# fgvieira/ngsDist

Hardware: AMD Instinct MI355X
Metric: pair-distances/sec (higher is better)
Workload: dtype f64

## Files before the change

include/ngsdist_amd.h:

```cpp
#ifndef NGSDIST_AMD_H
#define NGSDIST_AMD_H

#include <stdint.h>

#ifdef __cplusplus
extern "C" {
#endif

#define NGD_ABI_VERSION 6

#define NGD_OK 0
#define NGD_E_INVALID (-1)
#define NGD_E_NODEVICE (-2)
#define NGD_E_HIP (-3)
#define NGD_E_NOMEM (-4)
#define NGD_E_MODEL (-5)
#define NGD_E_NAN (-6)

#define NGD_KERNEL_AUTO 0
#define NGD_KERNEL_STREAM 1
#define NGD_KERNEL_MFMA 2
#define NGD_KERNEL_EM_FAITHFUL 3
#define NGD_KERNEL_EM_FAST 4
#define NGD_KERNEL_EM_TABLE 5
// ... 98 lines not shown
#define NGD_OPT_STAGE_RING 11
#define NGD_OPT_EAGER_FULL 12
#define NGD_OPT_WIN_PLAN 13
#define NGD_OPT_WIN_MAX_BYTES 14
#define NGD_OPT_EM_EXACT 15
#define NGD_OPT_EM_EXACT_CAP 16
#define NGD_OPT_UNIT_SKIP 17
#define NGD_OPT_EM_EXACT_WIN 18
#define NGD_OPT_NJ_MAX_BYTES 19
#define NGD_OPT_MDS_MAX_BYTES 20
#define NGD_OPT_DEBUG_FORGE_JOB 100
int ngd_set_option(ngd_engine *e, int option, uint64_t value);

int ngd_last_timing(const ngd_engine *e, ngd_timing *t);
int ngd_last_plain_pass(const ngd_engine *e, uint64_t *kgroups);
int ngd_image_mode(const ngd_engine *e, int *fixup);
typedef struct ngd_fixup_info {
  uint64_t flagged, recomputed, skipped;
  double ms;
  uint64_t by_pass;
} ngd_fixup_info;
int ngd_last_fixup(const ngd_engine *e, ngd_fixup_info *info);
typedef struct ngd_spill_timing {
  double ms_weights;
  double ms_terms;
  double ms_sanitize;
  double ms_contract;
  uint64_t chunks;
  uint64_t sites;
  uint64_t unit_sites;
// ... 183 lines not shown
```

ngsdist_amd/_lib.py:

```python
import ctypes as C
import os
import sys

_HERE = os.path.dirname(os.path.abspath(__file__))
LIB_PATH = os.environ.get("NGSDIST_AMD_LIB") or os.path.join(_HERE, "libngsdist_amd.so")


class NgdConfig(C.Structure):
    _fields_ = [
        ("n_ind", C.c_uint64),
        ("n_sites", C.c_uint64),
        ("score", C.c_double * 9),
        ("pairwise_del", C.c_int32),
        ("indep_geno", C.c_int32),
        ("device", C.c_int32),
        ("kernel", C.c_int32),
        ("shard_rank", C.c_uint32),
        ("shard_world", C.c_uint32),
        ("variant", C.c_uint32),
        ("n_slices", C.c_uint32),
        ("wg_target", C.c_uint32),
        ("exact_shapes", C.c_uint32),
        ("single_image", C.c_uint32),
        ("second_image_mib", C.c_uint32),
# ... 34 lines not shown

class NgdEmExactInfo(C.Structure):
    _fields_ = [("noted", C.c_uint64), ("changed", C.c_uint64), ("passes", C.c_uint64), ("ms", C.c_double)]


class NgdEmExactEntry(C.Structure):
    _fields_ = [("i1", C.c_uint32), ("i2", C.c_uint32), ("site", C.c_uint64), ("t_dev", C.c_uint32), ("t_ref", C.c_uint32),
                ("c_dev", C.c_double), ("c_ref", C.c_double)]


EXPORTS = [
    "ngd_last_error", "ngd_abi_version", "ngd_device_count", "ngd_create", "ngd_destroy",
    "ngd_upload_sites", "ngd_upload_ind_major", "ngd_commit", "ngd_stage_acquire", "ngd_stage_submit",
    "ngd_upload_raw_sites", "ngd_synth_fill", "ngd_synth_fill_range", "ngd_run", "ngd_run_mult", "ngd_run_mult_device",
    "ngd_run_device", "ngd_run_batch", "ngd_run_batch_device", "ngd_run_mult_batch",
    "ngd_run_mult_batch_device", "ngd_run_job", "ngd_run_job_device", "ngd_run_job_dist", "ngd_run_batch_dist", "ngd_run_mult_batch_dist", "ngd_fetch_matrix", "ngd_drop_caches", "ngd_set_option", "ngd_last_timing", "ngd_last_plain_pass", "ngd_last_spill_timing", "ngd_last_fixup", "ngd_image_mode", "ngd_last_shader_clock", "ngd_last_em_work", "ngd_finish", "ngd_finish_stream", "ngd_format_matrix", "ngd_taus_seed", "ngd_taus_get",
    "ngd_taus_uniform", "ngd_boot_block_map", "ngd_n_pairs", "ngd_pair_index", "ngd_device_bytes", "ngd_device_memory", "ngd_shard_of_pair", "ngd_shard_map",
    "ngd_score_congruence", "ngd_run_windows", "ngd_run_windows_device", "ngd_run_windows_dist", "ngd_last_windows",
    "ngd_window_ranges", "ngd_run_windows_job", "ngd_run_windows_job_device", "ngd_run_windows_job_dist",
    "ngd_window_ranges_bp", "ngd_window_boot_maps", "ngd_run_windows_job_var", "ngd_run_windows_job_var_device",
    "ngd_run_windows_job_var_dist",
    "ngd_last_em_exact", "ngd_em_exact_entries", "ngd_em2_site",
    "ngd_n_group_pairs", "ngd_group_pair_index", "ngd_group_cells", "ngd_set_groups", "ngd_group_means_device",
    "ngd_run_job_groups", "ngd_run_windows_groups", "ngd_run_windows_job_var_groups", "ngd_last_groups_ms",
    "ngd_boot_stats_max_rep", "ngd_boot_stats_host", "ngd_boot_stats_device", "ngd_boot_stats_values_device",
    "ngd_run_job_stats", "ngd_run_windows_job_var_stats", "ngd_run_job_groups_stats", "ngd_run_windows_job_var_groups_stats",
    "ngd_last_boot_stats_ms",
    "ngd_nj_max_ind", "ngd_nj_host", "ngd_nj_values_device", "ngd_nj_device", "ngd_run_job_nj", "ngd_run_windows_nj",
    "ngd_run_windows_job_var_nj", "ngd_last_nj_ms", "ngd_nj_support", "ngd_nj_newick",
    "ngd_mds_max_ind", "ngd_mds_max_dim", "ngd_mds_host", "ngd_mds_coords", "ngd_mds_values_device", "ngd_mds_device",
    "ngd_run_job_mds", "ngd_run_windows_mds", "ngd_run_windows_job_var_mds", "ngd_last_mds_ms",
# ... 46 lines not shown
    L.ngd_run_batch.argtypes = [vp, u64p, C.c_uint32, u64, u64, dp, u64p]
    L.ngd_run_batch_device.argtypes = [vp, u64p, C.c_uint32, u64, u64, vp, vp]
    L.ngd_run_mult_batch.argtypes = [vp, u32p, C.c_uint32, u64, u64, dp, u64p]
    L.ngd_run_job.argtypes = [vp, u64p, C.c_uint32, u64, u64, dp, u64p]
    L.ngd_run_job_device.argtypes = [vp, u64p, C.c_uint32, u64, u64, vp, vp]
    L.ngd_fetch_matrix.argtypes = [vp, C.c_uint32, dp, u64p]
    L.ngd_run_job_dist.argtypes = [vp, u64p, C.c_uint32, u64, u64, u64, u64, dp]
    L.ngd_run_batch_dist.argtypes = [vp, u64p, C.c_uint32, u64, u64, u64, u64, dp]
    L.ngd_run_mult_batch_dist.argtypes = [vp, u32p, C.c_uint32, u64, u64, u64, u64, dp]
    L.ngd_run_mult_batch_device.argtypes = [vp, u32p, C.c_uint32, u64, u64, vp, vp]
    L.ngd_drop_caches.argtypes = [vp]
    L.ngd_set_option.argtypes = [vp, C.c_int, u64]
    L.ngd_last_timing.argtypes = [vp, C.POINTER(NgdTiming)]
    if hasattr(L, "ngd_last_plain_pass"):
        L.ngd_last_plain_pass.argtypes = [vp, u64p]
    L.ngd_last_spill_timing.argtypes = [vp, C.POINTER(NgdSpillTiming)]
    L.ngd_last_fixup.argtypes = [vp, C.POINTER(NgdFixupInfo)]
    L.ngd_image_mode.argtypes = [vp, C.POINTER(C.c_int)]
    L.ngd_image_mode.restype = C.c_int
    L.ngd_last_em_work.argtypes = [vp, u64p, u64p]
    L.ngd_last_shader_clock.argtypes = [vp, dp]
    L.ngd_finish.argtypes = [dp, u64p, u64, u64, u64, dp]
    L.ngd_finish_stream.argtypes = [dp, u64p, u64, u64, u64, dp, u64p]
    L.ngd_format_matrix.argtypes = [dp, u64, C.POINTER(C.c_char_p), C.c_char_p, u64, C.c_uint32]
    L.ngd_format_matrix.restype = C.c_int64
    L.ngd_device_memory.argtypes = [C.c_int, u64p, u64p]
    L.ngd_taus_seed.argtypes = [u32p, u64]
    L.ngd_taus_seed.restype = None
    L.ngd_taus_get.argtypes = [u32p]
    L.ngd_taus_get.restype = C.c_uint32
# ... 93 lines not shown
```

ngsdist_amd/csrc/engine.hip:

```cpp
#include "ngd_engine.h"

extern "C" {

const char *ngd_last_error(void) { return g_err.c_str(); }
int ngd_abi_version(void) { return NGD_ABI_VERSION; }

uint64_t ngd_n_pairs(uint64_t n_ind) { return n_ind * (n_ind - 1) / 2; }
uint64_t ngd_pair_index(uint64_t n_ind, uint64_t i1, uint64_t i2) { return ngd_pair_idx(n_ind, i1, i2); }
uint64_t ngd_device_bytes(const ngd_engine *e) { return e ? e->dev_bytes : 0; }

int ngd_run_device(ngd_engine *e, const uint64_t *block_map, uint64_t n_blocks, uint64_t block_size,
                   void *d_sum, void *d_cnt) {
  if (!d_sum || !d_cnt) return fail(NGD_E_INVALID, "ngd_run_device: null output");
  return run_impl(e, block_map, nullptr, block_map ? 1 : 0, false, n_blocks, block_size, (double *)d_sum,
                  (unsigned long long *)d_cnt);
}

int ngd_run_mult_device(ngd_engine *e, const uint32_t *mult, uint64_t n_blocks, uint64_t block_size, void *d_sum,
                        void *d_cnt) {
  if (!d_sum || !d_cnt || !mult) return fail(NGD_E_INVALID, "ngd_run_mult_device: null argument");
  return run_impl(e, nullptr, mult, 1, false, n_blocks, block_size, (double *)d_sum, (unsigned long long *)d_cnt);
}

int ngd_run_mult(ngd_engine *e, const uint32_t *mult, uint64_t n_blocks, uint64_t block_size, double *sum,
// ... 115 lines not shown
      if (e->pin_sites || e->committed) return fail(NGD_E_INVALID, "ngd_set_option: NGD_OPT_EAGER_FULL before the first ngd_stage_acquire");
      if (value && e->opt_em_exact) return fail(NGD_E_INVALID, "ngd_set_option: NGD_OPT_EAGER_FULL and NGD_OPT_EM_EXACT refuse each other (the eager pass does not note)");
      e->opt_eager = value != 0 && eager_supported(e);
      break;
    case NGD_OPT_STAGE_PIECE_MIB:
    case NGD_OPT_STAGE_RING:
      if (e->pin_sites) return fail(NGD_E_INVALID, "ngd_set_option: the staging ring exists already (set before the first ngd_stage_acquire)");
      if (option == NGD_OPT_STAGE_RING) {
        if (value < 2 || value > ngd_engine::RING) return fail(NGD_E_INVALID, "ngd_set_option: NGD_OPT_STAGE_RING is 2 .. 8");
        e->opt_stage_ring = value;
      } else {
        if (value < 1 || value > 1024) return fail(NGD_E_INVALID, "ngd_set_option: NGD_OPT_STAGE_PIECE_MIB is 1 .. 1024");
        e->opt_stage_piece_mib = value;
      }
      break;
    case NGD_OPT_UNIT_SKIP: e->opt_unit_skip = value != 0; break;
    case NGD_OPT_DEBUG_FORGE_JOB: {
      const char *hook = getenv("NGD_ENABLE_TEST_HOOKS");
      if (!hook || strcmp(hook, "1") != 0)
        return fail(NGD_E_INVALID, "ngd_set_option: NGD_OPT_DEBUG_FORGE_JOB is a test hook (set NGD_ENABLE_TEST_HOOKS=1)");
      if (e->kernel != NGD_KERNEL_MFMA || !e->d_jobs) return fail(NGD_E_INVALID, "ngd_set_option: no MFMA job list");
      HIPCHK(hipSetDevice(e->device));
      ngd_job j;
      HIPCHK(hipMemcpy(&j, e->d_jobs, sizeof(j), hipMemcpyDeviceToHost));
      j.rows = (uint8_t)(value & 7); j.cols = (uint8_t)((value >> 3) & 7); j.tri = (uint8_t)((value >> 6) & 1);
      HIPCHK(hipMemcpy(e->d_jobs, &j, sizeof(j), hipMemcpyHostToDevice));
      break;
    }
    default: return fail(NGD_E_INVALID, "ngd_set_option: unknown option");
  }
  return NGD_OK;
// ... 32 lines not shown
  return e->congruent ? 2 : e->single_image ? 1 : 3;
}

int ngd_last_spill_timing(const ngd_engine *e, ngd_spill_timing *t) {
  if (!e || !t) return fail(NGD_E_INVALID, "ngd_last_spill_timing: null argument");
  *t = e->spill_timing;
  return NGD_OK;
}

int ngd_last_plain_pass(const ngd_engine *e, uint64_t *kgroups) {
  if (!e || !kgroups) return fail(NGD_E_INVALID, "ngd_last_plain_pass: null argument");
  *kgroups = e->plain_kg;
  return NGD_OK;
}

int ngd_last_timing(const ngd_engine *e, ngd_timing *t) {
  if (!e || !t) return fail(NGD_E_INVALID, "ngd_last_timing: null argument");
  *t = e->timing;
  return NGD_OK;
}

}
```

ngsdist_amd/csrc/engine_plans.hip:

```cpp
#include "ngd_engine.h"

struct pass_slices {
  const uint32_t *w = nullptr, *kgl = nullptr;
  uint64_t sites_eff = 0;
  uint32_t n_ks = 0;
  uint64_t per_slice = 0, kg_lim = 0;
  double *slab = nullptr;
  uint64_t k_per_slice = 0;
  uint32_t w_stride = 0;
  bool note = false;
  const uint64_t *seg = nullptr;
};

static ngd_mfma_launch slices_launch(const ngd_engine *e, const pass_slices &p, const double *d_w_plain) {
  ngd_mfma_launch l;
  l.PA = e->PA;
  l.d_wk = p.k_per_slice ? e->blk.wslice : (p.w ? e->d_wk : d_w_plain);
  l.n_ks = p.n_ks; l.kg_per_slice = p.per_slice; l.n_kg_eff = p.kg_lim;
  l.k_per_slice = p.k_per_slice; l.w_slice_stride = p.w_stride;
  if (p.seg) { l.d_wk = e->blk.wslice; l.d_seg = p.seg; l.w_slice_stride = 1; l.k_per_slice = 0; }
  l.slab = p.slab;
  return l;
}

// ... 232 lines not shown
  int rc = pass_once(e, mult, mult_max, n_blocks, block_size, n_drawn, d_sum, d_cnt, add_timing, note);
  if (rc || !note) return rc;
  bool again = false;
  if ((rc = em_exact_finish(e, d_sum, &again))) return rc;
  if (again) {
    if ((rc = pass_once(e, mult, mult_max, n_blocks, block_size, n_drawn, d_sum, d_cnt, add_timing, true))) return rc;
    if ((rc = em_exact_finish(e, d_sum, &again))) return rc;
    if (again) return fail(NGD_E_HIP, "NGD_OPT_EM_EXACT: internal -- the second pass noted more than the first counted");
    e->exact_info.passes = 2;
  }
  return NGD_OK;
}

static int partials_impl(ngd_engine *e, const uint32_t *mult , const unsigned long long *drawn,
                         uint32_t n_rep, uint64_t n_blocks, uint64_t block_size, double *d_sum,
                         unsigned long long *d_cnt, bool *feasible, bool note = false) {
  const ngd_geom &g = e->g;
  const uint64_t n_pairs = ngd_n_pairs(g.n_ind);
  const uint64_t n_eff = n_blocks * block_size;
  const uint64_t plane = (uint64_t)g.n_pad * g.n_pad;
  const bool mfma = e->kernel == NGD_KERNEL_MFMA;
  const bool pdel = e->cfg.pairwise_del != 0;
  *feasible = false;
  if (e->kernel == NGD_KERNEL_STREAM || !e->opt_boot_partials) return NGD_OK;
  const bool unaligned = mfma && block_size % 4 != 0;
  if (unaligned && !e->opt_boot_unaligned) return NGD_OK;
  if (n_blocks >= (1ull << 31)) return NGD_OK;
  const uint64_t unit = mfma ? 3 * block_size / 4 : block_size;
  const bool cached = !note && e->blk.has_sums(block_size, n_blocks);
  uint64_t sub = 1, nks = 0;
  if (cached) {
    sub = e->blk.sub;
    nks = e->blk.nks;
  } else {
    const uint32_t tiles_n = mfma ? std::max(1u, e->n_wg / (e->exact_shapes && e->exact_shapes < 3 ? 4 : 1))
                                  : e->kernel == NGD_KERNEL_EM_TABLE ? e->n_tiles64 : e->n_tiles16;
    const uint64_t want = e->opt_boot_wg;
    while (!unaligned && tiles_n && (uint64_t)tiles_n * n_blocks * sub < want && unit % (sub * 2) == 0 &&
           unit / (sub * 2) >= 32)
      sub *= 2;
    nks = n_blocks * sub;
    if (mfma) nks = (nks + 7) / 8 * 8;
  }
  if (nks >= (1ull << 31)) return NGD_OK;
  const uint64_t elems = nks * plane, c_elems = pdel ? n_blocks * plane : 0;
  const bool c_cached = !pdel || e->blk.has_counts(block_size, n_blocks);
  if (!cached || !c_cached) {
    size_t free_b = 0, total_b = 0;
    HIPCHK(hipMemGetInfo(&free_b, &total_b));
    const uint64_t need = elems * 8 + c_elems * 4;
    const uint64_t have = e->blk.bytes();
    const uint64_t budget = e->opt_boot_max_bytes ? e->opt_boot_max_bytes : (uint64_t)((free_b + have) / 100 * 85);
    if (need > budget) return NGD_OK;
// ... 20 lines not shown
  }
  *feasible = true;
  if (e->out.on && out_trace()) fprintf(stderr, "[out] plan settled %.3f ms into the call\n", out_now() - e->out.t_call);

  HIPCHK(hipEventRecord(e->ev[0], e->st));
  uint32_t launches = 0;
  HIPCHK(hipEventRecord(e->ev[1], e->st));
  if (!cached) {
    int rc = e->blk.borrow_sums().ensure(e, elems);
    if (rc) return rc;
    e->blk.nks = (uint32_t)nks;
    e->blk.sub = (uint32_t)sub;
    e->blk.per_slice = unit / sub;
    pass_slices ps;
    ps.sites_eff = n_eff; ps.n_ks = e->blk.nks; ps.slab = e->blk.sums();
    if (unaligned && e->congruent) {
      std::vector<uint64_t> tab;
      tab.reserve((size_t)e->blk.nks * NGD_SEG_STRIDE);
      uint64_t wkg = 0, max_wkg = 0;
      for (uint64_t b = 0; b < n_blocks; b++) {
        const uint64_t s_lo = b * block_size, s_hi = s_lo + block_size;
        const uint64_t kg0 = ngd_kg_lo(s_lo, 1), kg1 = ngd_kg_hi(s_hi, 1), n_wkg = kg1 - kg0 + 1 + NGD_KG_TAIL;
        tab.insert(tab.end(), {kg0, kg1, wkg, s_lo, s_hi});
        wkg += n_wkg;
        max_wkg = std::max(max_wkg, n_wkg);
      }
      for (uint64_t k = n_blocks; k < e->blk.nks; k++) tab.insert(tab.end(), {0, 0, wkg, 0, 0});
      max_wkg = std::max<uint64_t>(max_wkg, 1 + NGD_KG_TAIL);
      rc = e->blk.wslice.ensure(e, (wkg + 1 + NGD_KG_TAIL) * 4);
      if (!rc) rc = e->d_segtab.ensure(e, tab.size());
      if (rc) return rc;
      HIPCHK(hipMemcpy(e->d_segtab, tab.data(), tab.size() * 8, hipMemcpyHostToDevice));
      ngd_launch_seg_weights(e->st, e->d_segtab, e->blk.nks, max_wkg, e->sc.d, e->blk.wslice);
      ps.kg_lim = g.n_kg; ps.seg = e->d_segtab;
    } else if (unaligned) {
      const uint32_t w_stride = (uint32_t)((3 * block_size + 3) / 4 + 1 + NGD_KG_TAIL);
      rc = e->blk.wslice.ensure(e, (uint64_t)e->blk.nks * w_stride * 4);
      if (rc) return rc;
      ngd_launch_slice_weights(e->st, e->blk.nks, w_stride, 3 * block_size, 3 * n_eff, e->blk.wslice);
      ps.kg_lim = (3 * n_eff + 3) / 4; ps.k_per_slice = 3 * block_size; ps.w_stride = w_stride;
    } else {
      if (note && (rc = em_exact_begin(e))) return rc;
      ps.per_slice = e->blk.per_slice; ps.kg_lim = mfma ? 3 * n_eff / 4 : 0; ps.note = note;
    }
    rc = launch_accumulate(e, ps);
    if (rc) return rc;
    HIPCHK(hipGetLastError());
    if (!note) e->blk.sums_filled(block_size, n_blocks);
    launches = 1;
  }
  HIPCHK(hipEventRecord(e->ev[2], e->st));

  const uint32_t stride = (n_rep + ngd_reduce_chunk(n_rep) - 1) / ngd_reduce_chunk(n_rep) * ngd_reduce_chunk(n_rep);
  const uint64_t n_slices = n_blocks * sub;
  std::vector<double> W(n_slices * stride, 0.0);
  for (uint32_t r = 0; r < n_rep; r++)
    for (uint64_t b = 0; b < n_blocks; b++) {
      const double m = (double)mult[(uint64_t)r * n_blocks + b];
      if (m != 0.0)
        for (uint64_t q = 0; q < sub; q++) W[(b * sub + q) * stride + r] = m;
    }
  int rc = e->d_W.ensure(e, W.size());
  if (rc) return rc;
  HIPCHK(hipMemcpyAsync(e->d_W, W.data(), W.size() * 8, hipMemcpyHostToDevice, e->st));
  if ((rc = zero_outputs(e, n_rep, d_sum, d_cnt, false))) return rc;
  const bool fix = e->SM != nullptr && mfma;
  const ngd_fix_flags ff{e->d_fixlist, e->d_fixcount, e->d_fixseen, e->fix_cap};
  std::vector<double> thr;
  if (fix) {
    thr.resize(n_rep);
    for (uint32_t r = 0; r < n_rep; r++) thr[r] = NGD_FIX_MEAN * (double)drawn[r];
    rc = e->d_fixthr.ensure(e, (uint64_t)n_rep);
    if (rc) return rc;
    HIPCHK(hipMemcpyAsync(e->d_fixthr, thr.data(), (uint64_t)n_rep * 8, hipMemcpyHostToDevice, e->st));
    HIPCHK(hipMemsetAsync(e->d_fixcount, 0, sizeof(uint32_t), e->st));
    HIPCHK(hipMemsetAsync(e->d_fixseen, 0, (n_pairs / 32 + 1) * sizeof(uint32_t), e->st));
  }
  const bool fix_in_reduce = fix && !pdel;
  std::vector<uint32_t> M;
  auto counts_inputs = [&]() -> int {
    if (pdel) {
      if (!c_cached) {
        int rc = e->blk.borrow_counts().ensure(e, c_elems);
        if (rc) return rc;
        ngd_launch_count_blocks(e->st, g, e->mask, block_size, (uint32_t)n_blocks, e->d_tiles16, e->n_tiles16, e->blk.counts());
        HIPCHK(hipGetLastError());
// ... 51 lines not shown
    HIPCHK(hipEventRecord(e->ev[3], e->st));

    if ((rc = counts_inputs())) return rc;
    if (pdel) {
      ngd_launch_reduce_c(e->st, g, e->blk.counts(), (uint32_t)n_blocks, e->d_M, stride, n_rep, e->d_tiles, e->n_tiles, d_cnt);
      if (fix) {
        ngd_launch_fix_flag(e->st, g, d_sum, d_cnt, n_rep, e->d_tiles, e->n_tiles, ff);
        HIPCHK(hipMemcpyAsync(e->h_fixcount, e->d_fixcount, sizeof(uint32_t), hipMemcpyDeviceToHost, e->st));
      }
    }
  }
  HIPCHK(hipGetLastError());
  if (!stream_out) HIPCHK(hipEventRecord(e->ev[4], e->st));
  HIPCHK(hipStreamSynchronize(e->st));
  if (stream_out && out_trace()) fprintf(stderr, "[out] engine stream drained +%.3f\n", out_now() - e->out.t0);
  read_timing(e, n_eff, launches, false);
  if ((rc = mfma_fault(e))) return rc;
  if (fix) {
    bool patched = false;
    rc = fixup_pass(e, nullptr, n_eff, nullptr, block_size / sub, (uint32_t)n_slices, &patched);
    if (rc) return rc;
    if (patched) {
      if (stream_out && (rc = out_requeue(e))) return rc;
      ngd_launch_reduce_w(e->st, g, e->blk.sums(), (uint32_t)n_slices, e->d_W, stride, n_rep, e->d_tiles, e->n_tiles, d_sum);
      HIPCHK(hipGetLastError());
      HIPCHK(hipStreamSynchronize(e->st));
    }
  }
  return NGD_OK;
}

static int em_batch_impl(ngd_engine *e, const uint32_t *mult, const uint32_t *mult_max, const unsigned long long *drawn,
// ... 346 lines not shown
```

ngsdist_amd/csrc/layout.hip:

```cpp
#include <algorithm>

#include "ngd_internal.h"

namespace {

struct ngd_d3 {
  double v[3];
  int quad;
};
inline ngd_d3 d3_of(const double *d3) { return d3 ? ngd_d3{{d3[0], d3[1], d3[2]}, 1} : ngd_d3{{1.0, 1.0, 1.0}, 0}; }

__device__ __forceinline__ void emit(const ngd_geom &g, const ngd_score &sc, int pairwise_del,
                                     uint64_t s, uint32_t i, double p0, double p1, double p2,
                                     double *PA, double *QB, double *PI, unsigned long long *mask) {
  if (PI && !sc.congruent) {
    double *d = PI + (i * g.n_sites_pad + s) * 3;
    d[0] = p0; d[1] = p1; d[2] = p2;
  }
  bool miss = ngd_miss(p0, p1, p2);
  if (mask) {
    unsigned long long *w = &mask[(uint64_t)i * g.n_words + (s >> 6)];
    const unsigned long long bit = 1ull << (s & 63);
    if (miss) atomicAnd(w, ~bit);
    else atomicOr(w, bit);
// ... 350 lines not shown
  for (uint64_t q = q0; q < q1; q++) {
    const double v = T[(3 * q * g.n_ig + ig) * 64 + lane];
    const uint64_t s = 4 * q + (lane >> 4);
    if (s < g.n_sites && i < g.n_ind) {
      const double d = v - 1.0;
      if (!(__builtin_fabs(d) <= 0x1p-40)) bad = true;
      else acc += (long long)(d * 0x1p53);
    }
  }
  acc += __shfl_xor(acc, 16, 64);
  acc += __shfl_xor(acc, 32, 64);
  if (lane < 16 && i < g.n_ind && acc) atomicAdd((unsigned long long *)&E[i], (unsigned long long)acc);
  if (bad) atomicOr(flag, 1);
}

}

void ngd_launch_unit_scan(hipStream_t st, const ngd_geom &g, const double *T, long long *d_E, int *d_flag) {
  const uint64_t n_q = g.n_sites_pad >> 2;
  const uint64_t per_wg = std::max<uint64_t>(64, (n_q + 32767) / 32768);
  hipLaunchKernelGGL(k_unit_scan, dim3(g.n_ig / 4, (unsigned)((n_q + per_wg - 1) / per_wg)), dim3(256), 0, st, g, T, per_wg, d_E,
                     d_flag);
}

uint32_t ngd_kg_count_blocks(uint64_t n_kg) { return (uint32_t)((n_kg + CPB - 1) / CPB); }

void ngd_launch_kg_compact(hipStream_t st, const double *d_wk, uint64_t n_kg, uint32_t tail_kg, uint32_t *d_counts,
                           uint32_t *d_list) {
  const uint32_t nb = ngd_kg_count_blocks(n_kg);
  hipLaunchKernelGGL(k_kg_count, dim3(nb), dim3(256), 0, st, d_wk, n_kg, d_counts);
// ... 113 lines not shown
```

ngsdist_amd/csrc/ngd_engine.h:

```cpp
#pragma once
#include <algorithm>
#include <atomic>
#include <chrono>
#include <cmath>
#include <cstdio>
#include <cstdlib>
#include <cstring>
#include <condition_variable>
#include <functional>
#include <memory>
#include <mutex>
#include <string>
#include <thread>
#include <vector>

#include "kg_ranges.h"
#include "ngd_buffers.h"
#include "ngd_internal.h"
#include "ngd_shard.h"

#pragma GCC visibility push(hidden)


struct BlockScratch {
  DevBuf<double> wslice;
  uint64_t per_slice = 0;
  uint32_t nks = 0, sub = 0;
  bool has_sums(uint64_t B, uint64_t blocks) const { return boot_B == B && boot_blocks == blocks; }
  bool has_counts(uint64_t B, uint64_t blocks) const { return cnt_B == B && cnt_blocks == blocks; }
  uint64_t sums_block() const { return boot_B; }
  const DevBuf<double> &sums() const { return slab_boot; }
  const DevBuf<uint32_t> &counts() const { return cnt_boot; }
  DevBuf<double> &borrow_sums() { boot_B = boot_blocks = 0; return slab_boot; }
  DevBuf<uint32_t> &borrow_counts() { cnt_B = cnt_blocks = 0; return cnt_boot; }
  void sums_filled(uint64_t B, uint64_t blocks) { boot_B = B; boot_blocks = blocks; }
  void counts_filled(uint64_t B, uint64_t blocks) { cnt_B = B; cnt_blocks = blocks; }
  void drop() { boot_B = boot_blocks = cnt_B = cnt_blocks = 0; }
  uint64_t bytes() const { return slab_boot.bytes() + cnt_boot.bytes(); }

 private:
  DevBuf<double> slab_boot;
  DevBuf<uint32_t> cnt_boot;
  uint64_t boot_B = 0, boot_blocks = 0, cnt_B = 0, cnt_blocks = 0;
};

struct ngd_engine : ngd_mem {
  ngd_config cfg{};
  ngd_geom g{};
  ngd_score sc{};
  int kernel = 0;
  hipEvent_t ev[5] = {};
  DevBuf<double> PA, QB, PI;
  bool single_image = false;
  bool congruent = false;
  DevBuf<double> d_wD;
  DevBuf<uint32_t> d_kgskip;
  uint64_t n_kgskip = 0, skip_per_slice = 0;
  DevBuf<long long> d_unitE;
  bool unit_ok = false;
  uint64_t opt_unit_skip = 1;
  uint64_t plain_kg = 0;
  DevBuf<double> SM;
  DevBuf<unsigned long long> d_fixlist;
  DevBuf<uint32_t> d_fixcount, d_fixseen;
  PinBuf<uint32_t> h_fixcount;
  DevBuf<double> d_fixparts, d_fixthr;
  DevBuf<ngd_fix_tile> d_fixtiles;
  DevBuf<double> d_fixtparts;
  DevBuf<double> fix_p, fix_q, d_fixnew;
  ngd_fixup_info fix_info{};
  std::vector<ngd_tile> h_tiles16;
  uint32_t fix_cap = 0;
  uint64_t opt_fix_work = 0;
  DevBuf<double> QB_res;
  uint64_t qb_res_kg = 0;
  DevBuf<double> qb_chunk;
// ... 261 lines not shown
```

ngsdist_amd/csrc/ngd_internal.h:

```cpp
#pragma once
#include <hip/hip_runtime.h>
#include <stdint.h>

#include "../../include/ngsdist_amd.h"
#include "ngd_layout.h"
#include "win_plan.h"

#define NGD_TILE 128
#define NGD_IG 16
#define NGD_IG_PER_TILE (NGD_TILE / NGD_IG)
#define NGD_KG_TAIL 8
#define NGD_KG_LIST_PAD 16

typedef double ngd_d4 __attribute__((ext_vector_type(4)));

struct ngd_score {
  double v[9];
  double c[9], d[3];
  int congruent;
  int fix;
  double fix_sign;
};

struct ngd_geom {
// ... 50 lines not shown
void ngd_launch_synth(hipStream_t st, const ngd_geom &g, uint64_t seed, double miss_frac, uint64_t site0,
                      const ngd_score &score, int pairwise_del, double *PA, double *QB, double *PI,
                      unsigned long long *mask);
void ngd_launch_weights(hipStream_t st, uint64_t n_blocks, uint64_t block_size, uint64_t n_sites,
                        const uint32_t *d_mult, uint32_t *d_ws, double *d_wk, const double *d3 = nullptr);
uint32_t ngd_kg_count_blocks(uint64_t n_kg);
void ngd_launch_kg_compact(hipStream_t st, const double *d_wk, uint64_t n_kg, uint32_t tail_kg, uint32_t *d_counts,
                           uint32_t *d_list);
void ngd_launch_weights_batch(hipStream_t st, const uint32_t *d_mult, uint32_t n_rep, uint32_t rb, int lead_full,
                              uint64_t n_blocks, uint64_t block_size, uint64_t n_sites, uint64_t n_sites_alloc,
                              double *d_W);
void ngd_launch_slice_weights(hipStream_t st, uint32_t n_slices, uint32_t stride, uint64_t k_per_slice, uint64_t k_total,
                              double *d_W);
void ngd_launch_index_weights(hipStream_t st, uint64_t n_k, const double *d3, double *d_W);
void ngd_launch_unit_scan(hipStream_t st, const ngd_geom &g, const double *T, long long *d_E, int *d_flag);
void ngd_launch_planes(hipStream_t st, const uint32_t *d_ws, uint64_t n_sites, uint32_t n_words,
                       uint32_t n_planes, unsigned long long *d_planes);

void ngd_launch_accum_stream(hipStream_t st, const ngd_geom &g, const double *PI, const uint32_t *d_ws,
                             uint64_t n_sites_eff, const ngd_score &score, int pairwise_del,
                             const uint64_t *d_pairs, uint64_t n_owned, double *d_sum);

void ngd_launch_seg_weights(hipStream_t st, const uint64_t *d_seg, uint32_t n_seg, uint64_t max_wkg, const double *d3,
                            double *d_W);

struct ngd_mfma_engine {
  const ngd_geom &g;
  const ngd_job *d_jobs;
  uint32_t n_wg;
  int exact_shapes;
// ... 81 lines not shown
                               uint64_t n_eff, uint64_t n_blocks, uint64_t block_size, double *D);
void ngd_launch_contract(hipStream_t st, const double *d_Wt, const double *C, uint32_t n_mat, uint32_t n_pg, uint32_t n_kg,
                         double *D);
void ngd_launch_spill_scatter(hipStream_t st, const double *D, uint32_t n_pg, const ngd_tile *d_tiles64, uint32_t n_tiles64,
                              const uint32_t *d_rowpg, uint64_t n_ind, uint32_t n_mat, double *d_sum);

void ngd_launch_accum_em_table_slices(hipStream_t st, const ngd_emt_common &c, uint32_t ks0, uint32_t n_sub, uint64_t sites_per_slice,
                                      double *slab, uint32_t lds_pad);
void ngd_launch_accum_em_batch(hipStream_t st, const ngd_geom &g, const double *PA, const double *d_Wb, int rb,
                               uint64_t n_sites_eff, const ngd_score &score, int pairwise_del, int fast,
                               const ngd_tile *d_tiles16, uint32_t n_tiles16, uint32_t n_ks,
                               uint64_t sites_per_slice, double *slab);

#define NGD_FIX_MEAN 1e-6
#define NGD_FIX_MEAN_UNIT 1e-3
#define NGD_FIX_CAP 4096u
#define NGD_FIX_LIST (1u << 20)
#define NGD_FIX_TILE_COST_X10 43u
struct ngd_fix_flags {
  unsigned long long *list;
  uint32_t *count;
  uint32_t *seen;
  uint32_t cap;
};
struct ngd_fix_tile {
  uint16_t ig, jg;
  uint32_t n;
  unsigned long long mask[4];
};
#define NGD_FIX_TILE_MIN 5u
// ... 1 lines not shown
                            const uint32_t *d_ws, const ngd_fix_tile *d_tiles, uint32_t n_tiles, uint64_t s_lo, uint64_t s_hi,
                            uint64_t sites_per_slice, uint32_t n_slices, int out_mode, double *out);
void ngd_launch_fixup_tiles_finish(hipStream_t st, const ngd_geom &g, const ngd_fix_tile *d_tiles, uint32_t n_tiles,
                                   const double *parts, uint32_t n_slices, double *d_sum);
void ngd_launch_fixup(hipStream_t st, const ngd_geom &g, const ngd_score &score, const double *T, const double *SM,
                      const uint32_t *d_ws, const unsigned long long *d_list, uint32_t n_list, uint64_t s_lo, uint64_t s_hi,
                      uint64_t sites_per_slice, uint32_t n_slices, int out_mode, double *out);
void ngd_launch_fixup_finish(hipStream_t st, const ngd_geom &g, const unsigned long long *d_list, uint32_t n_list,
                             const double *parts, uint32_t n_slices, double *d_sum);

void ngd_launch_reduce(hipStream_t st, const ngd_geom &g, const double *slab, uint32_t n_ks,
                       uint32_t planes_per_slice, const ngd_tile *d_tiles, uint32_t n_tiles, double *d_sum,
                       unsigned long long *d_cnt = nullptr, unsigned long long cnt_value = 0,
                       const ngd_fix_flags *fix = nullptr, double fix_thr = 0, const long long *unit_E = nullptr,
                       double unit_c = 0, double unit_d0 = 0);
void ngd_launch_pq_range(hipStream_t st, const ngd_geom &g, const ngd_score &score, const double *T, const double *SM,
                         const uint32_t *d_ws, uint64_t kg_lo, uint64_t kg_end, double *Ps, double *Qs);
void ngd_launch_fix_merge(hipStream_t st, const ngd_geom &g, const double *d_new, double *d_sum, const unsigned long long *d_cnt,
                          double thr, const ngd_tile *d_tiles, uint32_t n_tiles);
void ngd_launch_fix_flag(hipStream_t st, const ngd_geom &g, const double *d_sum, const unsigned long long *d_cnt,
                         uint32_t n_rep, const ngd_tile *d_tiles, uint32_t n_tiles, const ngd_fix_flags &fix,
                         uint32_t mat_stride = 1 );
int ngd_finish_matrices_stream(const double *sum, const uint64_t *cnt, const uint64_t *cnt_mat, uint32_t n_mat, uint64_t n_pairs,
                               uint64_t evol_model, double *dist, const volatile uint64_t *landed);
uint32_t ngd_reduce_chunk(uint32_t n_rep);
void ngd_launch_reduce_w(hipStream_t st, const ngd_geom &g, const double *slab, uint32_t n_ks, const double *d_W,
                         uint32_t w_stride, uint32_t n_rep, const ngd_tile *d_tiles, uint32_t n_tiles,
                         double *d_sum, const ngd_fix_flags *fix = nullptr, const double *d_thr = nullptr, uint32_t chunk = 0);
void ngd_launch_reduce_c(hipStream_t st, const ngd_geom &g, const uint32_t *C, uint32_t n_blocks, const uint32_t *d_M,
                         uint32_t m_stride, uint32_t n_rep, const ngd_tile *d_tiles, uint32_t n_tiles,
// ... 81 lines not shown
```

ngsdist_amd/csrc/reduce.hip:

```cpp
#include <type_traits>

#include "ngd_internal.h"

namespace {

__device__ __forceinline__ bool ngd_finite(double v) { return __builtin_fabs(v) <= 1.7976931348623157e308; }

__global__ __launch_bounds__(128) void k_reduce(const double *__restrict__ slab, uint32_t n_ks,
                                                 uint32_t planes_per_slice, const ngd_tile *__restrict__ tiles,
                                                 uint32_t n_pad, uint64_t n_ind, double *__restrict__ d_sum,
                                                 unsigned long long *__restrict__ d_cnt, unsigned long long cnt_value,
                                                 ngd_fix_flags fix, double fix_thr, const long long *__restrict__ unit_E,
                                                 double unit_c, double unit_d0) {
  const uint32_t tile = blockIdx.x >> 7, row = blockIdx.x & 127;
  const uint32_t i = tiles[tile].ti * NGD_TILE + row;
  const uint32_t j = tiles[tile].tj * NGD_TILE + threadIdx.x;
  if (!(i < j && j < n_ind)) return;
  const uint64_t plane = (uint64_t)n_pad * n_pad * planes_per_slice;
  const double *p = slab + (uint64_t)i * n_pad + j;
  double s[8] = {0, 0, 0, 0, 0, 0, 0, 0};
  uint32_t ks = 0;
  for (; ks + 8 <= n_ks; ks += 8) {
#pragma unroll
    for (int u = 0; u < 8; u++) s[u] += p[(uint64_t)(ks + u) * plane];
  }
  for (int u = 0; ks < n_ks; ks++, u++) s[u] += p[(uint64_t)ks * plane];
  const uint64_t idx = ngd_pair_idx(n_ind, i, j);
  double sum = ((s[0] + s[1]) + (s[2] + s[3])) + ((s[4] + s[5]) + (s[6] + s[7]));
  if (unit_E) sum = (unit_c + sum) + unit_d0 * ((double)(unit_E[i] + unit_E[j]) * 0x1p-53);
  d_sum[idx] = sum;
  if (d_cnt) d_cnt[idx] = cnt_value;
  if (fix.list && sum < fix_thr) {
    const uint32_t slot = atomicAdd(fix.count, 1u);
    if (slot < fix.cap) fix.list[slot] = ((unsigned long long)i << 32) | j;
  }
}

template <int RB>
__global__ __launch_bounds__(128) void k_reduce_wb(const double *__restrict__ slab, uint32_t n_ks,
                                                    const double *__restrict__ W, uint32_t w_stride,
                                                    uint32_t n_rep, const ngd_tile *__restrict__ tiles,
                                                    uint32_t n_pad, uint64_t n_ind, uint64_t n_pairs,
                                                    double *__restrict__ d_sum, ngd_fix_flags fix,
                                                    const double *__restrict__ fix_thr) {
  const uint32_t tile = blockIdx.x >> 7, row = blockIdx.x & 127;
  const uint32_t i = tiles[tile].ti * NGD_TILE + row;
  const uint32_t j = tiles[tile].tj * NGD_TILE + threadIdx.x;
  if (!(i < j && j < n_ind)) return;
  const uint32_t r0 = blockIdx.y * RB;
// ... 557 lines not shown
                     n_blocks, d_M, m_stride, n_rep, d_tiles, g.n_pad, g.n_ind, g.n_ind * (g.n_ind - 1) / 2, d_cnt);
}

}

void ngd_launch_reduce(hipStream_t st, const ngd_geom &g, const double *slab, uint32_t n_ks,
                       uint32_t planes_per_slice, const ngd_tile *d_tiles, uint32_t n_tiles, double *d_sum,
                       unsigned long long *d_cnt, unsigned long long cnt_value, const ngd_fix_flags *fix, double fix_thr,
                       const long long *unit_E, double unit_c, double unit_d0) {
  if (!n_tiles) return;
  hipLaunchKernelGGL(k_reduce, dim3(n_tiles * NGD_TILE), dim3(128), 0, st, slab, n_ks, planes_per_slice, d_tiles,
                     g.n_pad, g.n_ind, d_sum, d_cnt, cnt_value, fix ? *fix : ngd_fix_flags{nullptr, nullptr, nullptr, 0}, fix_thr,
                     unit_E, unit_c, unit_d0);
}

void ngd_launch_fix_flag(hipStream_t st, const ngd_geom &g, const double *d_sum, const unsigned long long *d_cnt,
                         uint32_t n_rep, const ngd_tile *d_tiles, uint32_t n_tiles, const ngd_fix_flags &fix, uint32_t mat_stride) {
  if (!n_tiles || !n_rep) return;
  hipLaunchKernelGGL(k_fix_flag, dim3(n_tiles * NGD_TILE), dim3(128), 0, st, d_sum, d_cnt, n_rep, d_tiles, g.n_ind,
                     ngd_n_pairs(g.n_ind) * mat_stride, NGD_FIX_MEAN, fix);
}

void ngd_launch_fix_merge(hipStream_t st, const ngd_geom &g, const double *d_new, double *d_sum, const unsigned long long *d_cnt,
                          double thr, const ngd_tile *d_tiles, uint32_t n_tiles) {
  if (!n_tiles) return;
  hipLaunchKernelGGL(k_fix_merge, dim3(n_tiles * NGD_TILE), dim3(128), 0, st, d_new, d_sum, d_cnt, thr, NGD_FIX_MEAN, d_tiles,
                     g.n_ind);
}

uint32_t ngd_reduce_chunk(uint32_t n_rep) { return n_rep <= 1 ? 1 : n_rep <= 4 ? 4 : n_rep <= 16 ? 16 : 32; }
// ... 188 lines not shown
```

ngsdist_amd/engine.py:

```python
import ctypes as C

import numpy as np

from . import _lib

KERNELS = {"auto": 0, "stream": 1, "mfma": 2, "em_faithful": 3, "em_fast": 4, "em_table": 5}
OPTIONS = {"boot_partials": 1, "boot_max_bytes": 2, "boot_wg": 3, "boot_unaligned": 4, "em_batch": 5,
           "em_spill": 6, "em_spill_bytes": 7, "single_image_bytes": 8, "fixup_work": 9, "stage_piece_mib": 10,
           "stage_ring": 11, "eager_full": 12, "win_plan": 13, "win_max_bytes": 14, "em_exact": 15, "em_exact_cap": 16,
           "unit_skip": 17, "em_exact_win": 18, "nj_max_bytes": 19, "mds_max_bytes": 20,
           "debug_forge_job": 100}
EM_EXACT_ENTRY = np.dtype([("i1", np.uint32), ("i2", np.uint32), ("site", np.uint64), ("t_dev", np.uint32),
                           ("t_ref", np.uint32), ("c_dev", np.float64), ("c_ref", np.float64)], align=True)

DEFAULT_SCORE = (0.0, 0.5, 1.0, 0.5, 0.0, 0.5, 1.0, 0.5, 0.0)


class NgdError(RuntimeError):
    def __init__(self, code, msg):
        super().__init__("ngsdist_amd error %d: %s" % (code, msg))
        self.code = code


def _check(rc):
# ... 534 lines not shown
    def set_option(self, name, value):
        _check(self._L.ngd_set_option(self._h, OPTIONS[name], int(value)))
        return self

    def drop_caches(self):
        _check(self._L.ngd_drop_caches(self._h))

    def timing(self):
        t = _lib.NgdTiming()
        _check(self._L.ngd_last_timing(self._h, C.byref(t)))
        return {k: getattr(t, k) for k, _ in t._fields_}

    def plain_pass_kgroups(self):
        n = C.c_uint64(0)
        _check(self._L.ngd_last_plain_pass(self._h, C.byref(n)))
        return int(n.value)

    def spill_timing(self):
        t = _lib.NgdSpillTiming()
        _check(self._L.ngd_last_spill_timing(self._h, C.byref(t)))
        return {k: getattr(t, k) for k, _ in t._fields_}

    def image_mode(self):
        f = C.c_int(0)
        m = self._L.ngd_image_mode(self._h, C.byref(f))
        return int(m), bool(f.value)

    def fixup(self):
        t = _lib.NgdFixupInfo()
        _check(self._L.ngd_last_fixup(self._h, C.byref(t)))
# ... 331 lines not shown
```

Baseline: 16.00 million.

## Extend unit-site skipping to bootstrap partials via per-slice scan and fold

Applies the existing unit-site skip (compacted k-group list) to the per-block bootstrap partials pass. The accumulation visits only non-unit k-groups, and a per-slice unit scan plus a fold kernel add back the unit-site contribution from integer-accumulated deviations. This is meant to cut MFMA work on the partials path when many sites are unit. In exchange it adds two extra kernels and a looser fixup threshold, and falls back to a full recompute when flagged pairs appear.

```diff
diff --git a/include/ngsdist_amd.h b/include/ngsdist_amd.h
--- a/include/ngsdist_amd.h
+++ b/include/ngsdist_amd.h
@@ -136,6 +136,7 @@
 
 int ngd_last_timing(const ngd_engine *e, ngd_timing *t);
 int ngd_last_plain_pass(const ngd_engine *e, uint64_t *kgroups);
+int ngd_last_partials_pass(const ngd_engine *e, uint64_t *kgroups);
 int ngd_image_mode(const ngd_engine *e, int *fixup);
 typedef struct ngd_fixup_info {
   uint64_t flagged, recomputed, skipped;
diff --git a/ngsdist_amd/_lib.py b/ngsdist_amd/_lib.py
--- a/ngsdist_amd/_lib.py
+++ b/ngsdist_amd/_lib.py
@@ -72,7 +72,7 @@
     "ngd_upload_sites", "ngd_upload_ind_major", "ngd_commit", "ngd_stage_acquire", "ngd_stage_submit",
     "ngd_upload_raw_sites", "ngd_synth_fill", "ngd_synth_fill_range", "ngd_run", "ngd_run_mult", "ngd_run_mult_device",
     "ngd_run_device", "ngd_run_batch", "ngd_run_batch_device", "ngd_run_mult_batch",
-    "ngd_run_mult_batch_device", "ngd_run_job", "ngd_run_job_device", "ngd_run_job_dist", "ngd_run_batch_dist", "ngd_run_mult_batch_dist", "ngd_fetch_matrix", "ngd_drop_caches", "ngd_set_option", "ngd_last_timing", "ngd_last_plain_pass", "ngd_last_spill_timing", "ngd_last_fixup", "ngd_image_mode", "ngd_last_shader_clock", "ngd_last_em_work", "ngd_finish", "ngd_finish_stream", "ngd_format_matrix", "ngd_taus_seed", "ngd_taus_get",
+    "ngd_run_mult_batch_device", "ngd_run_job", "ngd_run_job_device", "ngd_run_job_dist", "ngd_run_batch_dist", "ngd_run_mult_batch_dist", "ngd_fetch_matrix", "ngd_drop_caches", "ngd_set_option", "ngd_last_timing", "ngd_last_plain_pass", "ngd_last_partials_pass", "ngd_last_spill_timing", "ngd_last_fixup", "ngd_image_mode", "ngd_last_shader_clock", "ngd_last_em_work", "ngd_finish", "ngd_finish_stream", "ngd_format_matrix", "ngd_taus_seed", "ngd_taus_get",
     "ngd_taus_uniform", "ngd_boot_block_map", "ngd_n_pairs", "ngd_pair_index", "ngd_device_bytes", "ngd_device_memory", "ngd_shard_of_pair", "ngd_shard_map",
     "ngd_score_congruence", "ngd_run_windows", "ngd_run_windows_device", "ngd_run_windows_dist", "ngd_last_windows",
     "ngd_window_ranges", "ngd_run_windows_job", "ngd_run_windows_job_device", "ngd_run_windows_job_dist",
@@ -149,6 +149,8 @@
     L.ngd_last_timing.argtypes = [vp, C.POINTER(NgdTiming)]
     if hasattr(L, "ngd_last_plain_pass"):
         L.ngd_last_plain_pass.argtypes = [vp, u64p]
+    if hasattr(L, "ngd_last_partials_pass"):
+        L.ngd_last_partials_pass.argtypes = [vp, u64p]
     L.ngd_last_spill_timing.argtypes = [vp, C.POINTER(NgdSpillTiming)]
     L.ngd_last_fixup.argtypes = [vp, C.POINTER(NgdFixupInfo)]
     L.ngd_image_mode.argtypes = [vp, C.POINTER(C.c_int)]
diff --git a/ngsdist_amd/csrc/engine.hip b/ngsdist_amd/csrc/engine.hip
--- a/ngsdist_amd/csrc/engine.hip
+++ b/ngsdist_amd/csrc/engine.hip
@@ -153,7 +153,10 @@
         e->opt_stage_piece_mib = value;
       }
       break;
-    case NGD_OPT_UNIT_SKIP: e->opt_unit_skip = value != 0; break;
+    case NGD_OPT_UNIT_SKIP:
+      if (e->opt_unit_skip != (uint64_t)(value != 0) && e->blk.skipped) e->blk.borrow_sums();
+      e->opt_unit_skip = value != 0;
+      break;
     case NGD_OPT_DEBUG_FORGE_JOB: {
       const char *hook = getenv("NGD_ENABLE_TEST_HOOKS");
       if (!hook || strcmp(hook, "1") != 0)
@@ -216,6 +219,12 @@
   return NGD_OK;
 }
 
+int ngd_last_partials_pass(const ngd_engine *e, uint64_t *kgroups) {
+  if (!e || !kgroups) return fail(NGD_E_INVALID, "ngd_last_partials_pass: null argument");
+  *kgroups = e->partials_kg;
+  return NGD_OK;
+}
+
 int ngd_last_timing(const ngd_engine *e, ngd_timing *t) {
   if (!e || !t) return fail(NGD_E_INVALID, "ngd_last_timing: null argument");
   *t = e->timing;
diff --git a/ngsdist_amd/csrc/engine_plans.hip b/ngsdist_amd/csrc/engine_plans.hip
--- a/ngsdist_amd/csrc/engine_plans.hip
+++ b/ngsdist_amd/csrc/engine_plans.hip
@@ -270,7 +270,7 @@
 
 static int partials_impl(ngd_engine *e, const uint32_t *mult , const unsigned long long *drawn,
                          uint32_t n_rep, uint64_t n_blocks, uint64_t block_size, double *d_sum,
-                         unsigned long long *d_cnt, bool *feasible, bool note = false) {
+                         unsigned long long *d_cnt, bool *feasible, bool note = false, bool add_timing = false) {
   const ngd_geom &g = e->g;
   const uint64_t n_pairs = ngd_n_pairs(g.n_ind);
   const uint64_t n_eff = n_blocks * block_size;
@@ -283,8 +283,12 @@
   if (unaligned && !e->opt_boot_unaligned) return NGD_OK;
   if (n_blocks >= (1ull << 31)) return NGD_OK;
   const uint64_t unit = mfma ? 3 * block_size / 4 : block_size;
+  const bool skip_ok = mfma && !note && !pdel && !unaligned && e->congruent && !e->single_image && e->d_kgskip && e->unit_ok &&
+                       e->opt_unit_skip;
+  if (e->blk.skipped && !(e->unit_ok && e->opt_unit_skip)) e->blk.borrow_sums();
   const bool cached = !note && e->blk.has_sums(block_size, n_blocks);
   uint64_t sub = 1, nks = 0;
+  unit_partials_plan up;
   if (cached) {
     sub = e->blk.sub;
     nks = e->blk.nks;
@@ -292,7 +296,14 @@
     const uint32_t tiles_n = mfma ? std::max(1u, e->n_wg / (e->exact_shapes && e->exact_shapes < 3 ? 4 : 1))
                                   : e->kernel == NGD_KERNEL_EM_TABLE ? e->n_tiles64 : e->n_tiles16;
     const uint64_t want = e->opt_boot_wg;
-    while (!unaligned && tiles_n && (uint64_t)tiles_n * n_blocks * sub < want && unit % (sub * 2) == 0 &&
+    if (skip_ok) {
+      const uint64_t s = unit_partials_sub(block_size, n_blocks, tiles_n, want);
+      if (unit_partials_make(block_size, n_blocks, s, e->n_kgskip, NGD_UNIT_SKIP_MAX_SLICE_SITES, &up) &&
+          up.n_slices * (uint64_t)(g.n_ig >> 2) >= (1ull << 31))
+        up = unit_partials_plan{};
+    }
+    if (up.sub) sub = up.sub;
+    while (!up.sub && !unaligned && tiles_n && (uint64_t)tiles_n * n_blocks * sub < want && unit % (sub * 2) == 0 &&
            unit / (sub * 2) >= 32)
       sub *= 2;
     nks = n_blocks * sub;
@@ -343,14 +354,17 @@
     e->blk.per_slice = unit / sub;
     pass_slices ps;
     ps.sites_eff = n_eff; ps.n_ks = e->blk.nks; ps.slab = e->blk.sums();
+    e->partials_kg = mfma ? 3 * n_eff / 4 : 0;
+    if (up.sub && (rc = e->d_unitEs.ensure(e, up.n_slices * (uint64_t)g.n_ig * 16))) return rc;
     if (unaligned && e->congruent) {
       std::vector<uint64_t> tab;
       tab.reserve((size_t)e->blk.nks * NGD_SEG_STRIDE);
-      uint64_t wkg = 0, max_wkg = 0;
+      uint64_t wkg = 0, max_wkg = 0, visited = 0;
       for (uint64_t b = 0; b < n_blocks; b++) {
         const uint64_t s_lo = b * block_size, s_hi = s_lo + block_size;
         const uint64_t kg0 = ngd_kg_lo(s_lo, 1), kg1 = ngd_kg_hi(s_hi, 1), n_wkg = kg1 - kg0 + 1 + NGD_KG_TAIL;
         tab.insert(tab.end(), {kg0, kg1, wkg, s_lo, s_hi});
+        visited += kg1 - kg0;
         wkg += n_wkg;
         max_wkg = std::max(max_wkg, n_wkg);
       }
@@ -362,20 +376,35 @@
       HIPCHK(hipMemcpy(e->d_segtab, tab.data(), tab.size() * 8, hipMemcpyHostToDevice));
       ngd_launch_seg_weights(e->st, e->d_segtab, e->blk.nks, max_wkg, e->sc.d, e->blk.wslice);
       ps.kg_lim = g.n_kg; ps.seg = e->d_segtab;
+      e->partials_kg = visited;
     } else if (unaligned) {
       const uint32_t w_stride = (uint32_t)((3 * block_size + 3) / 4 + 1 + NGD_KG_TAIL);
       rc = e->blk.wslice.ensure(e, (uint64_t)e->blk.nks * w_stride * 4);
       if (rc) return rc;
       ngd_launch_slice_weights(e->st, e->blk.nks, w_stride, 3 * block_size, 3 * n_eff, e->blk.wslice);
       ps.kg_lim = (3 * n_eff + 3) / 4; ps.k_per_slice = 3 * block_size; ps.w_stride = w_stride;
+      e->partials_kg = 0;
+      for (uint64_t b = 0; b < n_blocks; b++)
+        e->partials_kg += std::min(ps.kg_lim, ((b + 1) * ps.k_per_slice + 3) >> 2) - ((b * ps.k_per_slice) >> 2);
     } else {
       if (note && (rc = em_exact_begin(e))) return rc;
       ps.per_slice = e->blk.per_slice; ps.kg_lim = mfma ? 3 * n_eff / 4 : 0; ps.note = note;
+      if (up.sub) {
+        ps.kgl = e->d_kgskip; ps.per_slice = up.list_per_slice; ps.kg_lim = up.list_lim;
+        e->partials_kg = up.list_lim;
+      }
     }
     rc = launch_accumulate(e, ps);
     if (rc) return rc;
     HIPCHK(hipGetLastError());
+    if (up.sub) {
+      ngd_launch_unit_scan_slices(e->st, g, e->PA, up.periods_per_slice, (uint32_t)up.n_slices, e->d_unitEs);
+      ngd_launch_unit_fold(e->st, g, e->blk.sums(), (uint32_t)up.n_slices, e->d_tiles, e->n_tiles, e->d_unitEs,
+                           e->sc.d[0] * (double)up.sites_per_slice, e->sc.d[0]);
+      HIPCHK(hipGetLastError());
+    }
     if (!note) e->blk.sums_filled(block_size, n_blocks);
+    e->blk.skipped = up.sub != 0;
     launches = 1;
   }
   HIPCHK(hipEventRecord(e->ev[2], e->st));
@@ -398,7 +427,8 @@
   std::vector<double> thr;
   if (fix) {
     thr.resize(n_rep);
-    for (uint32_t r = 0; r < n_rep; r++) thr[r] = NGD_FIX_MEAN * (double)drawn[r];
+    const double fix_mean = e->blk.skipped ? NGD_FIX_MEAN_UNIT : NGD_FIX_MEAN;
+    for (uint32_t r = 0; r < n_rep; r++) thr[r] = fix_mean * (double)drawn[r];
     rc = e->d_fixthr.ensure(e, (uint64_t)n_rep);
     if (rc) return rc;
     HIPCHK(hipMemcpyAsync(e->d_fixthr, thr.data(), (uint64_t)n_rep * 8, hipMemcpyHostToDevice, e->st));
@@ -480,8 +510,18 @@
   if (!stream_out) HIPCHK(hipEventRecord(e->ev[4], e->st));
   HIPCHK(hipStreamSynchronize(e->st));
   if (stream_out && out_trace()) fprintf(stderr, "[out] engine stream drained +%.3f\n", out_now() - e->out.t0);
-  read_timing(e, n_eff, launches, false);
+  read_timing(e, n_eff, launches, add_timing);
   if ((rc = mfma_fault(e))) return rc;
+  if (e->blk.skipped && fix && *(volatile uint32_t *)e->h_fixcount) {
+    e->unit_ok = false;
+    e->blk.borrow_sums();
+    if (stream_out) {
+      if ((rc = out_requeue(e))) return rc;
+      e->out.n_used = 0;
+      e->out.n_chunk_seq = 0;
+    }
+    return partials_impl(e, mult, drawn, n_rep, n_blocks, block_size, d_sum, d_cnt, feasible, note, true);
+  }
   if (fix) {
     bool patched = false;
     rc = fixup_pass(e, nullptr, n_eff, nullptr, block_size / sub, (uint32_t)n_slices, &patched);
diff --git a/ngsdist_amd/csrc/layout.hip b/ngsdist_amd/csrc/layout.hip
--- a/ngsdist_amd/csrc/layout.hip
+++ b/ngsdist_amd/csrc/layout.hip
@@ -388,6 +388,34 @@
   if (bad) atomicOr(flag, 1);
 }
 
+__global__ __launch_bounds__(256) void k_unit_scan_slices(ngd_geom g, const double *__restrict__ T, uint64_t per_slice,
+                                                          uint32_t n_slices, long long *__restrict__ E) {
+  const uint32_t wave = threadIdx.x >> 6, lane = threadIdx.x & 63;
+  const uint32_t n_q4 = g.n_ig >> 2;
+  const uint32_t slice = blockIdx.x / n_q4;
+  const uint32_t ig = (blockIdx.x % n_q4) * 4 + wave;
+  if (slice >= n_slices) return;
+  const uint32_t i = ig * 16 + (lane & 15);
+  const uint64_t q0 = (uint64_t)slice * per_slice, q1 = q0 + per_slice;
+  const uint64_t stride = 3 * (uint64_t)g.n_ig * 64;
+  const double *p = T + (3 * q0 * g.n_ig + ig) * 64 + lane;
+  long long acc = 0;
+#pragma unroll 8
+  for (uint64_t q = q0; q < q1; q++, p += stride) {
+    const double v = *p;
+    if (i < g.n_ind) acc += (long long)((v - 1.0) * 0x1p53);
+  }
+  acc += __shfl_xor(acc, 16, 64);
+  acc += __shfl_xor(acc, 32, 64);
+  if (lane < 16) E[(uint64_t)slice * g.n_ig * 16 + i] = acc;
+}
+
+}
+
+void ngd_launch_unit_scan_slices(hipStream_t st, const ngd_geom &g, const double *T, uint64_t periods_per_slice, uint32_t n_slices,
+                                 long long *d_E) {
+  if (!n_slices) return;
+  hipLaunchKernelGGL(k_unit_scan_slices, dim3(n_slices * (g.n_ig >> 2)), dim3(256), 0, st, g, T, periods_per_slice, n_slices, d_E);
 }
 
 void ngd_launch_unit_scan(hipStream_t st, const ngd_geom &g, const double *T, long long *d_E, int *d_flag) {
diff --git a/ngsdist_amd/csrc/ngd_engine.h b/ngsdist_amd/csrc/ngd_engine.h
--- a/ngsdist_amd/csrc/ngd_engine.h
+++ b/ngsdist_amd/csrc/ngd_engine.h
@@ -18,6 +18,7 @@
 #include "ngd_buffers.h"
 #include "ngd_internal.h"
 #include "ngd_shard.h"
+#include "unit_partials_plan.h"
 
 #pragma GCC visibility push(hidden)
 
@@ -26,16 +27,17 @@
   DevBuf<double> wslice;
   uint64_t per_slice = 0;
   uint32_t nks = 0, sub = 0;
+  bool skipped = false;
   bool has_sums(uint64_t B, uint64_t blocks) const { return boot_B == B && boot_blocks == blocks; }
   bool has_counts(uint64_t B, uint64_t blocks) const { return cnt_B == B && cnt_blocks == blocks; }
   uint64_t sums_block() const { return boot_B; }
   const DevBuf<double> &sums() const { return slab_boot; }
   const DevBuf<uint32_t> &counts() const { return cnt_boot; }
-  DevBuf<double> &borrow_sums() { boot_B = boot_blocks = 0; return slab_boot; }
+  DevBuf<double> &borrow_sums() { boot_B = boot_blocks = 0; skipped = false; return slab_boot; }
   DevBuf<uint32_t> &borrow_counts() { cnt_B = cnt_blocks = 0; return cnt_boot; }
   void sums_filled(uint64_t B, uint64_t blocks) { boot_B = B; boot_blocks = blocks; }
   void counts_filled(uint64_t B, uint64_t blocks) { cnt_B = B; cnt_blocks = blocks; }
-  void drop() { boot_B = boot_blocks = cnt_B = cnt_blocks = 0; }
+  void drop() { boot_B = boot_blocks = cnt_B = cnt_blocks = 0; skipped = false; }
   uint64_t bytes() const { return slab_boot.bytes() + cnt_boot.bytes(); }
 
  private:
@@ -60,6 +62,8 @@
   bool unit_ok = false;
   uint64_t opt_unit_skip = 1;
   uint64_t plain_kg = 0;
+  DevBuf<long long> d_unitEs;
+  uint64_t partials_kg = 0;
   DevBuf<double> SM;
   DevBuf<unsigned long long> d_fixlist;
   DevBuf<uint32_t> d_fixcount, d_fixseen;
diff --git a/ngsdist_amd/csrc/ngd_internal.h b/ngsdist_amd/csrc/ngd_internal.h
--- a/ngsdist_amd/csrc/ngd_internal.h
+++ b/ngsdist_amd/csrc/ngd_internal.h
@@ -88,6 +88,8 @@
                               double *d_W);
 void ngd_launch_index_weights(hipStream_t st, uint64_t n_k, const double *d3, double *d_W);
 void ngd_launch_unit_scan(hipStream_t st, const ngd_geom &g, const double *T, long long *d_E, int *d_flag);
+void ngd_launch_unit_scan_slices(hipStream_t st, const ngd_geom &g, const double *T, uint64_t periods_per_slice, uint32_t n_slices,
+                                 long long *d_E);
 void ngd_launch_planes(hipStream_t st, const uint32_t *d_ws, uint64_t n_sites, uint32_t n_words,
                        uint32_t n_planes, unsigned long long *d_planes);
 
@@ -199,6 +201,7 @@
 
 #define NGD_FIX_MEAN 1e-6
 #define NGD_FIX_MEAN_UNIT 1e-3
+#define NGD_UNIT_SKIP_MAX_SLICE_SITES 137488ull
 #define NGD_FIX_CAP 4096u
 #define NGD_FIX_LIST (1u << 20)
 #define NGD_FIX_TILE_COST_X10 43u
@@ -230,6 +233,8 @@
                        unsigned long long *d_cnt = nullptr, unsigned long long cnt_value = 0,
                        const ngd_fix_flags *fix = nullptr, double fix_thr = 0, const long long *unit_E = nullptr,
                        double unit_c = 0, double unit_d0 = 0);
+void ngd_launch_unit_fold(hipStream_t st, const ngd_geom &g, double *slab, uint32_t n_ks, const ngd_tile *d_tiles, uint32_t n_tiles,
+                          const long long *d_E, double unit_c, double unit_d0);
 void ngd_launch_pq_range(hipStream_t st, const ngd_geom &g, const ngd_score &score, const double *T, const double *SM,
                          const uint32_t *d_ws, uint64_t kg_lo, uint64_t kg_end, double *Ps, double *Qs);
 void ngd_launch_fix_merge(hipStream_t st, const ngd_geom &g, const double *d_new, double *d_sum, const unsigned long long *d_cnt,
diff --git a/ngsdist_amd/csrc/reduce.hip b/ngsdist_amd/csrc/reduce.hip
--- a/ngsdist_amd/csrc/reduce.hip
+++ b/ngsdist_amd/csrc/reduce.hip
@@ -1,3 +1,4 @@
+#include <algorithm>
 #include <type_traits>
 
 #include "ngd_internal.h"
@@ -33,6 +34,36 @@
   if (fix.list && sum < fix_thr) {
     const uint32_t slot = atomicAdd(fix.count, 1u);
     if (slot < fix.cap) fix.list[slot] = ((unsigned long long)i << 32) | j;
+  }
+}
+
+__global__ __launch_bounds__(128) void k_unit_fold(double *__restrict__ slab, uint32_t n_ks, const ngd_tile *__restrict__ tiles,
+                                                    uint32_t n_pad, uint64_t n_ind, const long long *__restrict__ E,
+                                                    uint32_t e_stride, double unit_c, double unit_d0) {
+  const uint32_t tile = blockIdx.x >> 7, row = blockIdx.x & 127;
+  const uint32_t i = tiles[tile].ti * NGD_TILE + row;
+  const uint32_t j = tiles[tile].tj * NGD_TILE + threadIdx.x;
+  if (!(i < j && j < n_ind)) return;
+  const uint64_t plane = (uint64_t)n_pad * n_pad;
+  double *p = slab + (uint64_t)i * n_pad + j;
+  constexpr int U = 4;
+  const uint32_t step = gridDim.y;
+  uint32_t ks = blockIdx.y;
+  for (; (uint64_t)ks + (uint64_t)(U - 1) * step < n_ks; ks += U * step) {
+    double v[U];
+    long long c[U];
+#pragma unroll
+    for (int u = 0; u < U; u++) {
+      const uint32_t s = ks + u * step;
+      v[u] = p[(uint64_t)s * plane];
+      c[u] = E[(uint64_t)s * e_stride + i] + E[(uint64_t)s * e_stride + j];
+    }
+#pragma unroll
+    for (int u = 0; u < U; u++) p[(uint64_t)(ks + u * step) * plane] = (unit_c + v[u]) + unit_d0 * ((double)c[u] * 0x1p-53);
+  }
+  for (; ks < n_ks; ks += step) {
+    const long long c = E[(uint64_t)ks * e_stride + i] + E[(uint64_t)ks * e_stride + j];
+    p[(uint64_t)ks * plane] = (unit_c + p[(uint64_t)ks * plane]) + unit_d0 * ((double)c * 0x1p-53);
   }
 }
 
@@ -620,6 +651,14 @@
                      unit_E, unit_c, unit_d0);
 }
 
+void ngd_launch_unit_fold(hipStream_t st, const ngd_geom &g, double *slab, uint32_t n_ks, const ngd_tile *d_tiles, uint32_t n_tiles,
+                          const long long *d_E, double unit_c, double unit_d0) {
+  if (!n_tiles || !n_ks) return;
+  const uint32_t ny = std::min<uint32_t>(65535u, std::max<uint32_t>(1u, (n_ks + 15) / 16));
+  hipLaunchKernelGGL(k_unit_fold, dim3(n_tiles * NGD_TILE, ny), dim3(128), 0, st, slab, n_ks, d_tiles, g.n_pad, g.n_ind, d_E,
+                     g.n_ig * 16u, unit_c, unit_d0);
+}
+
 void ngd_launch_fix_flag(hipStream_t st, const ngd_geom &g, const double *d_sum, const unsigned long long *d_cnt,
                          uint32_t n_rep, const ngd_tile *d_tiles, uint32_t n_tiles, const ngd_fix_flags &fix, uint32_t mat_stride) {
   if (!n_tiles || !n_rep) return;
diff --git a/ngsdist_amd/csrc/unit_partials_plan.h b/ngsdist_amd/csrc/unit_partials_plan.h
--- /dev/null
+++ b/ngsdist_amd/csrc/unit_partials_plan.h
@@ -0,0 +1,50 @@
+#pragma once
+#include <stdint.h>
+
+struct unit_partials_plan {
+  uint64_t sub = 0;
+  uint64_t n_slices = 0;
+  uint64_t periods_per_slice = 0;
+  uint64_t list_per_slice = 0;
+  uint64_t sites_per_slice = 0;
+  uint64_t list_lim = 0;
+};
+
+#define NGD_UNIT_PARTIALS_MIN_LIST 32
+
+inline uint64_t unit_partials_sub(uint64_t block_size, uint64_t n_blocks, uint64_t wg_per_slice, uint64_t want) {
+  const uint64_t periods = block_size / 4;
+  uint64_t sub = 1;
+  while (wg_per_slice && wg_per_slice * n_blocks * sub < want && periods % (sub * 2) == 0 &&
+         2 * periods / (sub * 2) >= NGD_UNIT_PARTIALS_MIN_LIST)
+    sub *= 2;
+  return sub;
+}
+
+inline bool unit_partials_make(uint64_t block_size, uint64_t n_blocks, uint64_t sub, uint64_t n_list, uint64_t max_slice_sites,
+                               unit_partials_plan *p) {
+  *p = unit_partials_plan{};
+  if (!block_size || !n_blocks || !sub || block_size % 4) return false;
+  const uint64_t periods = block_size / 4;
+  if (periods % sub) return false;
+  if (n_blocks > (1ull << 31) / sub) return false;
+  unit_partials_plan q;
+  q.sub = sub;
+  q.n_slices = n_blocks * sub;
+  q.periods_per_slice = periods / sub;
+  q.list_per_slice = 2 * q.periods_per_slice;
+  q.sites_per_slice = 4 * q.periods_per_slice;
+  if (q.sites_per_slice > max_slice_sites) return false;
+  if (q.n_slices > n_list / q.list_per_slice) return false;
+  q.list_lim = q.n_slices * q.list_per_slice;
+  *p = q;
+  return true;
+}
+
+inline void unit_partials_slice(const unit_partials_plan &p, uint64_t s, uint64_t *list_lo, uint64_t *list_hi, uint64_t *q_lo,
+                                uint64_t *q_hi) {
+  *q_lo = s * p.periods_per_slice;
+  *q_hi = *q_lo + p.periods_per_slice;
+  *list_lo = s * p.list_per_slice;
+  *list_hi = *list_lo + p.list_per_slice;
+}
diff --git a/ngsdist_amd/engine.py b/ngsdist_amd/engine.py
--- a/ngsdist_amd/engine.py
+++ b/ngsdist_amd/engine.py
@@ -572,6 +572,11 @@
     def plain_pass_kgroups(self):
         n = C.c_uint64(0)
         _check(self._L.ngd_last_plain_pass(self._h, C.byref(n)))
+        return int(n.value)
+
+    def partials_pass_kgroups(self):
+        n = C.c_uint64(0)
+        _check(self._L.ngd_last_partials_pass(self._h, C.byref(n)))
         return int(n.value)
 
     def spill_timing(self):
```

Result: no change. 16.02 million (median of 3 runs) (+0.1%).
